# MyrtleSoftware/myrtlespeech

Measured on AMD Instinct MI355X. Metric: audio-sec/s (RTF), DS2 5xBiLSTM-1024 encoder forward + CTC greedy, 80-feature 10 s clips @ batch 32/GPU, higher is better.
Workload: dtype f16x3 (f32 split in fp16 hi+lo, 3 fp16 MFMA passes, f32 acc: LSTM, projections, conv1/2, FC1; FC2/CTC/decode f32)

## Files before the change

### include/ms_hotpath.h

```cpp
#ifndef MS_HOTPATH_H
#define MS_HOTPATH_H

#include <stddef.h>
#include <stdint.h>

#ifdef __cplusplus
extern "C" {
#endif

#define MS_ABI_VERSION 4

enum {
  MS_OK = 0,
  MS_ERR_INVALID = 1,
  MS_ERR_HIP = 2,
  MS_ERR_WORKSPACE = 3,
  MS_ERR_TIMEOUT = 4,
  MS_ERR_UNSUPPORTED = 5
};

enum { MS_CELL_LSTM = 0, MS_CELL_GRU = 1, MS_CELL_RNN_TANH = 2, MS_CELL_HARD_LSTM = 3 };

enum { MS_ACT_NONE = 0, MS_ACT_CLAMP = 1  };

int ms_abi_version(void);
const char* ms_last_error(void);


int ms_mask_time_(float* x, const int32_t* lens, int N, int inner, int T, void* stream);

size_t ms_maskconv_packed_bytes(int Cout, int Cin_g, int KF, int KT, int groups);

int ms_maskconv_pack(const float* w, void* packed, int Cout, int Cin_g, int KF, int KT, int groups, void* stream);

int ms_maskconv_forward(const float* x, const int32_t* lens, const void* packed_w, const float* bias, float* y,
                        int N, int Cin, int Fin, int Tin, int Cout, int Fout, int Tout, int KF, int KT, int SF,
                        int ST, int DF, int DT, int pad_f_l, int pad_t_l, int groups, int act, float act_lo,
                        float act_hi, void* stream);

size_t ms_maskconv_cl_packed_bytes(int Cout, int Cin, int KF, int KT);
int ms_maskconv_cl_pack(const float* w, void* packed, int Cout, int Cin, int KF, int KT, void* stream);
size_t ms_maskconv_cl_workspace_bytes(int N, int Cin, int Fin, int Tin);
int ms_maskconv_cl_forward(const float* x, const int32_t* lens, const void* packed_w, const float* bias, float* y,
                           int N, int Cin, int Fin, int Tin, int Cout, int Fout, int Tout, int KF, int KT, int SF,
                           int ST, int DF, int DT, int pad_f_l, int pad_t_l, int act, float act_lo, float act_hi,
                           void* workspace, size_t workspace_bytes, void* stream);

size_t ms_maskconv_fwin_packed_bytes(int Cout, int KF, int KT);
int ms_maskconv_fwin_pack(const float* w, void* packed, int Cout, int KF, int KT, void* stream);
size_t ms_maskconv_fwin_workspace_bytes(int N, int Tin, int KF, int SF, int Fout);
int ms_maskconv_fwin_forward(const float* x, const int32_t* lens, const void* packed_w, const float* bias, float* y, int N,
                             int Fin, int Tin, int Cout, int Fout, int Tout, int KF, int KT, int SF, int ST, int DT,
                             int pad_f_l, int pad_t_l, int act, float act_lo, float act_hi, void* workspace,
                             size_t workspace_bytes, void* stream);

size_t ms_maskconv1d_gemm_packed_bytes(int Cout, int Cin, int KT);
int ms_maskconv1d_gemm_pack(const float* w, void* packed, int Cout, int Cin, int KT, void* stream);
size_t ms_maskconv1d_gemm_workspace_bytes(int N, int Cin, int Tout, int Cout, int KT);
int ms_maskconv1d_gemm_forward(const float* x, const int32_t* lens, const void* packed, const float* bias, float* y, int N,
                               int Cin, int Tin, int Cout, int Tout, int KT, int ST, int DT, int pad_l, int act,
                               float act_lo, float act_hi, void* workspace, size_t workspace_bytes, void* stream);

int ms_nct_to_tnc(const float* x, float* y, int N, int CF, int T, void* stream);

int ms_clamp(const float* x, float* y, size_t n, float lo, float hi, void* stream);


int ms_linear_forward(const float* x, const float* w, const float* bias, float* y, int M, int K, int N, int act,
                      float act_lo, float act_hi, void* stream);

#define MS_LINEAR_FEW_ROWS 1
size_t ms_linear_splitk_workspace_bytes(int M, int K, int N, int flags);
int ms_linear_splitk_forward(const float* x, const float* w, const float* bias, float* y, int M, int K, int N, int act,
                             float act_lo, float act_hi, int flags, void* workspace, size_t workspace_bytes, void* stream);

size_t ms_linear_split_workspace_bytes(int M, int K, int N);
int ms_linear_split_forward(const float* x, const float* w, const float* bias, float* y, int M, int K, int N, int act,
                            float act_lo, float act_hi, void* workspace, size_t workspace_bytes, void* stream);

size_t ms_linear_split_packed_bytes(int K, int N);
int ms_linear_split_pack(const float* w, void* packed, int K, int N, void* stream);
int ms_linear_split_forward_packed(const float* x, const void* packed_w, const float* bias, float* y, int M, int K, int N, int act,
                                   float act_lo, float act_hi, void* workspace, size_t workspace_bytes, void* stream);


int ms_lookahead_forward(const float* x, const float* w, float* y, int N, int F, int T, int ctx, long xs_n,
                         long xs_f, long xs_t, long ys_n, long ys_f, long ys_t, int act, float act_lo,
                         float act_hi, void* stream);

int ms_lookahead_window_forward(const float* x, const float* w, float* y, int N, int F, int T_in, int T_out, int ctx,
                                long xs_n, long xs_f, long xs_t, long ys_n, long ys_f, long ys_t, int act, float act_lo,
                                float act_hi, void* stream);


int ms_rnn_padded_hidden(int cell, int H, int ndir);
size_t ms_rnn_packed_bytes(int cell, int In, int H, int ndir);
int ms_rnn_pack(int cell, int In, int H, int ndir, const float* const* w_ih_host, const float* const* w_hh_host,
                const float* const* b_ih_host, const float* const* b_hh_host, void* packed, void* stream);

size_t ms_rnn_workspace_bytes(int cell, int T, int N, int In, int H, int ndir);

int ms_rnn_layer_forward(int cell, const void* packed, const float* x, const int32_t* lens, int max_len,
                         const float* h0, const float* c0, float* out, float* hn, float* cn, int T, int N, int In,
                         int H, int ndir, void* workspace, size_t workspace_bytes, void* stream);

enum { MS_RNN_X_PLANES_IN_WS = 1, MS_RNN_OUT_PLANES_TO_WS = 2, MS_RNN_PACKED_ROWS = 4, MS_RNN_HX_PREINIT = 4096,
       MS_RNN_RECURRENCE_ONLY = 8192, MS_RNN_TIMING_SKIP_PROJECTION = 8192 ,
       MS_RNN_PROJECTION_ONLY = 16384 };
int ms_rnn_layer_chains_planes(int cell, int H, int ndir);
int ms_rnn_hx_preinit(int cell, int T, int N, int In, int H, int ndir, int max_len, int nregions, void* workspace,
                      size_t workspace_bytes, void* stream);
int ms_rnn_layer_packs_rows(int cell, int T, int N, int In, int H, int ndir);
int ms_rnn_layer_forward_ex(int cell, const void* packed, const float* x, const int32_t* lens, int max_len,
                            const float* h0, const float* c0, float* out, float* hn, float* cn, int T, int N, int In,
                            int H, int ndir, int flags, void* workspace, size_t workspace_bytes, void* stream);

int ms_rnn_layer_is_wide(int cell, int H, int ndir, int N);
int ms_rnn_stack_overlap_ok(int cell, int T, int N, int In, int H, int ndir, int nl);
int ms_rnn_stack_forward(int cell, const void* const* packed_host, const float* x, const int32_t* lens, int max_len,
                         const float* h0, const float* c0, float* out, float* hn, float* cn, int T, int N, int In, int H, int ndir,
                         int nl, int segments, void* workspace, size_t workspace_bytes, void* stream);

int ms_rnn_status(const void* workspace, void* stream);

size_t ms_rnn_debug_offset(int cell, int T, int N, int In, int H, int ndir);

int ms_gemm_set_variant(int variant);

enum {
  MS_PROF_PROJECTION = 0, MS_PROF_RECURRENCE = 1, MS_PROF_GEMM_K_LARGE = 2, MS_PROF_GEMM_K_SMALL = 3, MS_PROF_CONV = 4,
  MS_PROF_LAYOUT = 5, MS_PROF_LINEAR = 6, MS_PROF_GREEDY = 7, MS_PROF_OTHER = 8
};
#define MS_PROF_KINDS 9
int ms_prof_enable(int on);
int ms_prof_read(float* out_ms_host, int* out_n_host);

int ms_clock_probe(unsigned long long* out_dev, int samples, int spacing_us, void* stream);
// ... 105 lines not shown
```

### myrtlespeech_amd/_lib.py

```python
import ctypes
import os
import re
from ctypes import POINTER, c_char_p, c_double, c_float, c_int, c_int32, c_long, c_size_t, c_void_p

import torch

_HERE = os.path.dirname(os.path.abspath(__file__))
LIB_PATH = os.environ.get("MS_HOTPATH_LIB") or os.path.join(_HERE, "libms_hotpath.so")
HEADER_PATH = os.path.join(os.path.dirname(_HERE), "include", "ms_hotpath.h")

MS_OK = 0
ABI_VERSION = 4
ERR_NAMES = {1: "MS_ERR_INVALID", 2: "MS_ERR_HIP", 3: "MS_ERR_WORKSPACE", 4: "MS_ERR_TIMEOUT", 5: "MS_ERR_UNSUPPORTED"}

CELL_LSTM, CELL_GRU, CELL_RNN_TANH, CELL_HARD_LSTM = 0, 1, 2, 3
ACT_NONE, ACT_CLAMP = 0, 1
LINEAR_FEW_ROWS = 1
PROF_KINDS = 9

_P = c_void_p
_PP = POINTER(c_void_p)

SIGNATURES = {
    "ms_abi_version": (c_int, []),
    "ms_last_error": (c_char_p, []),
    "ms_mask_time_": (c_int, [_P, _P, c_int, c_int, c_int, _P]),
    "ms_maskconv_packed_bytes": (c_size_t, [c_int, c_int, c_int, c_int, c_int]),
    "ms_maskconv_pack": (c_int, [_P, _P, c_int, c_int, c_int, c_int, c_int, _P]),
    "ms_maskconv_forward": (c_int, [_P, _P, _P, _P, _P] + [c_int] * 17 + [c_float, c_float, _P]),
    "ms_maskconv_cl_packed_bytes": (c_size_t, [c_int, c_int, c_int, c_int]),
    "ms_maskconv_cl_pack": (c_int, [_P, _P, c_int, c_int, c_int, c_int, _P]),
    "ms_maskconv_cl_workspace_bytes": (c_size_t, [c_int, c_int, c_int, c_int]),
    "ms_maskconv_cl_forward": (c_int, [_P, _P, _P, _P, _P] + [c_int] * 16 + [c_float, c_float, _P, c_size_t, _P]),
    "ms_maskconv_fwin_packed_bytes": (c_size_t, [c_int, c_int, c_int]),
    "ms_maskconv_fwin_pack": (c_int, [_P, _P, c_int, c_int, c_int, _P]),
    "ms_maskconv_fwin_workspace_bytes": (c_size_t, [c_int, c_int, c_int, c_int, c_int]),
    "ms_maskconv_fwin_forward": (c_int, [_P, _P, _P, _P, _P] + [c_int] * 14 + [c_float, c_float, _P, c_size_t, _P]),
    "ms_maskconv1d_gemm_packed_bytes": (c_size_t, [c_int, c_int, c_int]),
    "ms_maskconv1d_gemm_pack": (c_int, [_P, _P, c_int, c_int, c_int, _P]),
    "ms_maskconv1d_gemm_workspace_bytes": (c_size_t, [c_int] * 5),
    "ms_maskconv1d_gemm_forward": (c_int, [_P, _P, _P, _P, _P] + [c_int] * 10 + [c_float, c_float, _P, c_size_t, _P]),
    "ms_nct_to_tnc": (c_int, [_P, _P, c_int, c_int, c_int, _P]),
    "ms_clamp": (c_int, [_P, _P, c_size_t, c_float, c_float, _P]),
    "ms_linear_forward": (c_int, [_P, _P, _P, _P, c_int, c_int, c_int, c_int, c_float, c_float, _P]),
    "ms_linear_splitk_workspace_bytes": (c_size_t, [c_int, c_int, c_int, c_int]),
    "ms_linear_splitk_forward": (c_int, [_P, _P, _P, _P, c_int, c_int, c_int, c_int, c_float, c_float, c_int, _P, c_size_t, _P]),
    "ms_linear_split_workspace_bytes": (c_size_t, [c_int, c_int, c_int]),
    "ms_linear_split_forward": (c_int, [_P, _P, _P, _P, c_int, c_int, c_int, c_int, c_float, c_float, _P, c_size_t, _P]),
    "ms_linear_split_packed_bytes": (c_size_t, [c_int, c_int]),
    "ms_linear_split_pack": (c_int, [_P, _P, c_int, c_int, _P]),
    "ms_linear_split_forward_packed": (c_int, [_P, _P, _P, _P, c_int, c_int, c_int, c_int, c_float, c_float, _P, c_size_t, _P]),
    "ms_lookahead_forward": (c_int, [_P, _P, _P, c_int, c_int, c_int, c_int] + [c_long] * 6 + [c_int, c_float, c_float, _P]),
    "ms_lookahead_window_forward": (c_int, [_P, _P, _P, c_int, c_int, c_int, c_int, c_int] + [c_long] * 6 + [c_int, c_float, c_float, _P]),
    "ms_rnn_packed_bytes": (c_size_t, [c_int, c_int, c_int, c_int]),
    "ms_ctc_status": (c_int, [_P, _P]),
    "ms_rnn_padded_hidden": (c_int, [c_int, c_int, c_int]),
    "ms_rnn_hx_preinit": (c_int, [c_int] * 8 + [_P, c_size_t, _P]),
    "ms_rnn_pack": (c_int, [c_int, c_int, c_int, c_int, _PP, _PP, _PP, _PP, _P, _P]),
    "ms_rnn_workspace_bytes": (c_size_t, [c_int] * 6),
    "ms_rnn_layer_forward": (c_int, [c_int, _P, _P, _P, c_int, _P, _P, _P, _P, _P] + [c_int] * 5 + [_P, c_size_t, _P]),
    "ms_rnn_layer_forward_ex": (c_int, [c_int, _P, _P, _P, c_int, _P, _P, _P, _P, _P] + [c_int] * 6 + [_P, c_size_t, _P]),
    "ms_rnn_layer_chains_planes": (c_int, [c_int, c_int, c_int]),
    "ms_rnn_layer_is_wide": (c_int, [c_int] * 4),
    "ms_rnn_stack_overlap_ok": (c_int, [c_int] * 7),
    "ms_rnn_stack_forward": (c_int, [c_int, _P, _P, _P, c_int, _P, _P, _P, _P, _P] + [c_int] * 7 + [_P, c_size_t, _P]),
    "ms_rnn_status": (c_int, [_P, _P]),
    "ms_rnn_debug_offset": (c_size_t, [c_int] * 6),
    "ms_rnn_layer_packs_rows": (c_int, [c_int] * 6),
    "ms_gemm_set_variant": (c_int, [c_int]),
    "ms_prof_enable": (c_int, [c_int]),
    "ms_prof_read": (c_int, [POINTER(c_float), POINTER(c_int)]),
    "ms_clock_probe": (c_int, [_P, c_int, c_int, _P]),
    "ms_barrier_chain_probe": (c_int, [_P, c_int, c_int, _P]),
    "ms_ctc_loss_workspace_bytes": (c_size_t, [c_int] * 4),
    "ms_ctc_loss_forward": (c_int, [_P] * 7 + [c_int] * 7 + [_P, c_size_t, _P]),
    "ms_log_softmax_axis": (c_int, [_P, _P, c_int, c_int, c_int, _P]),
    "ms_log_softmax_axis_backward": (c_int, [_P, _P, _P, c_int, c_int, c_int, _P]),
    "ms_ctc_loss_backward_workspace_bytes": (c_size_t, [c_int] * 4),
    "ms_ctc_loss_backward": (c_int, [_P] * 7 + [c_int] * 6 + [_P, c_size_t, _P]),
    "ms_ctc_greedy_decode": (c_int, [_P, _P, _P, _P, c_int, c_int, c_int, c_int, _P]),
    "ms_ctc_greedy_stream_state_bytes": (c_size_t, [c_int]),
    "ms_ctc_greedy_stream_begin": (c_int, [_P, c_int, _P]),
    "ms_ctc_greedy_stream_step": (c_int, [_P, c_int, c_int, c_int, c_int, _P, _P, _P, _P, c_int, _P, _P, c_int, _P]),
    "ms_embedding_forward": (c_int, [_P, _P, _P, c_int, c_int, c_int, _P]),
    "ms_rnnt_joint_forward": (c_int, [_P, _P, _P, _P, _P, _P, c_int, c_int, c_int, _P]),
    "ms_rnnt_topk": (c_int, [_P, _P, _P, c_int, c_int, c_int, _P]),
    "ms_ctc_beam_workspace_bytes": (c_size_t, [c_int] * 4),
    "ms_ctc_beam_decode": (c_int, [_P, _P, _P, _P, c_int, c_int, c_int, c_int, c_int, c_float, c_int, _P, c_int, c_int,
                                   _P, c_int, _P, _P, _P, _P, c_size_t, _P]),
    "ms_ctc_beam_decode_rows": (c_int, [_P, _P, _P, _P, c_int, c_int, c_int, c_int, c_int, c_float, c_int, _P, c_int, c_int,
                                        c_int, c_int, _P, c_int, _P, _P, _P, _P, c_size_t, _P]),
    "ms_ngram_lm_table_check": (c_int, [_P, c_size_t]),
    "ms_ngram_lm_score": (c_int, [_P, _P, c_size_t, _P, _P, _P, c_int, c_int, c_int, _P]),
    "ms_ctc_beam_lm_workspace_bytes": (c_size_t, [c_int] * 5),
    "ms_ctc_beam_decode_lm": (c_int, [_P, _P, _P, _P, c_int, c_int, c_int, c_int, c_int, c_float, c_int, _P, c_int, c_int,
                                      c_int, c_int, _P, _P, c_size_t, c_int, _P, _P, _P, _P, c_size_t, _P]),
    "ms_rnnt_decode_workspace_bytes": (c_size_t, [c_int] * 10),
    "ms_rnnt_decode": (c_int, [_P, _P, _P, _PP, _PP, _PP, _PP, _P, _P, _P, _P, _P, _P] + [c_int] * 10 + [_P, c_size_t, _P]),
    "ms_mfcc_workspace_bytes": (c_size_t, [c_int] * 5),
    "ms_mfcc_forward": (c_int, [_P] * 7 + [c_int] * 7 + [c_float, _P, c_size_t, _P]),
    "ms_mfcc_legacy_forward": (c_int, [_P] * 7 + [c_int] * 8 + [c_double, _P]),
    "ms_standardize_workspace_bytes": (c_size_t, [c_int]),
    "ms_standardize_forward": (c_int, [_P, _P, _P, c_int, c_int, c_int, _P, c_size_t, _P]),
    "ms_context_frames_forward": (c_int, [_P, _P, _P, c_int, c_int, c_int, c_int, _P]),
    "ms_spec_augment_": (c_int, [_P, _P, _P] + [c_int] * 6 + [_P]),
}

_lib = None


def header_symbols():
    with open(HEADER_PATH) as f:
        text = re.sub(r"/\*.*?\*/", "", f.read(), flags=re.S)
    return sorted(set(re.findall(r"\b(ms_[a-z0-9_]+)\s*\(", text)))


# ... 194 lines not shown
```

### myrtlespeech_amd/csrc/conv_cl.hip

```cpp
#include <algorithm>
#include <type_traits>

#include "common.h"

namespace {

typedef unsigned u32x4 __attribute__((ext_vector_type(4)));
typedef unsigned u32x2 __attribute__((ext_vector_type(2)));
typedef __bf16 bf16x8 __attribute__((ext_vector_type(8)));
typedef _Float16 f16x8 __attribute__((ext_vector_type(8)));

constexpr int CL_F = 2;

struct ClP {
  int N, Cin, Fin, Tin, Cout, Fout, Tout, KF, KT, SF, ST, DF, DT, pad_f, pad_t;
  int KG;
  int PW;
  int co_tiles;
  int act;
  float lo, hi;
  int FP;
};

__device__ __forceinline__ unsigned bf16b(float x) { return (unsigned)__builtin_bit_cast(unsigned short, (__bf16)x); }
// ... 71 lines not shown
      const bool frow = (fo0 + f) < p.Fout && (WIN || (fin >= 0 && fin < p.Fin));
      const size_t rbase = ((size_t)n * p.Fin + (frow && !WIN ? fin : 0)) * p.Tin;
      for (int i = tid; i < ngran; i += 256) {
        const int q = i / p.KG, kg = i - q * p.KG;
        const int tin = tin0 + q;
        u32x4 vh = {0u, 0u, 0u, 0u}, vl = {0u, 0u, 0u, 0u};
        if (frow && tin >= 0 && tin < len) {
          if (WIN) {
            const int boff = (int)((((size_t)n * p.Tin + tin) * p.FP + (size_t)(fo0 + f) * p.SF + kg * 8) * 2);
            vh = __builtin_amdgcn_raw_buffer_load_b128(xh_rsrc, boff, 0, 0);
            if (!F16) vl = __builtin_amdgcn_raw_buffer_load_b128(xl_rsrc, boff, 0, 0);
          } else {
            const size_t off = (rbase + tin) * p.Cin + kg * 8;
            vh = *reinterpret_cast<const u32x4*>(xh + off);
            if (!F16) vl = *reinterpret_cast<const u32x4*>(xl + off);
          }
        }
        *reinterpret_cast<u32x4*>(Ph + f * row_bytes + (kg * p.PW + q) * 16) = vh;
        if (!F16) *reinterpret_cast<u32x4*>(Pl + f * row_bytes + (kg * p.PW + q) * 16) = vl;
      }
    }
    const int taps_per_stage = (p.KT + 1) / 2;
    for (int kt0 = 0; kt0 < p.KT; kt0 += taps_per_stage) {
      const int ntap = min(taps_per_stage, p.KT - kt0);
      if (kt0 > 0) __syncthreads();
      {
        const int ng = ntap * p.KG * 32;
        for (int i = tid; i < ng; i += 256) {
          const int co = i & 31, rest = i >> 5;
          const size_t src = ((((size_t)kf * p.KT + kt0) * p.KG + rest) * cout_pad + tile * 32 + co) * 8;
          *reinterpret_cast<u32x4*>(Wh + i * 16) = *reinterpret_cast<const u32x4*>(wp + src);
          if (!F16) *reinterpret_cast<u32x4*>(Wl + i * 16) = *reinterpret_cast<const u32x4*>(wp + wplane + src);
        }
      }
      __syncthreads();
      for (int ktl = 0; ktl < ntap; ++ktl) {
        const int tq = (wt * 32 + l31) * p.ST + (kt0 + ktl) * p.DT;
        for (int s = 0; s < p.KG / 2; ++s) {
          const int kg = 2 * s + half;
          const int woff = ((ktl * p.KG + kg) * 32 + l31) * 16;
          const u32x4 ah = *reinterpret_cast<const u32x4*>(Wh + woff);
          u32x4 al = ah;
          if (!F16) al = *reinterpret_cast<const u32x4*>(Wl + woff);
#pragma unroll
          for (int f = 0; f < CL_F; ++f) {
            const int poff = (wf * CL_F + f) * row_bytes + (kg * p.PW + tq) * 16;
            const u32x4 bh = *reinterpret_cast<const u32x4*>(Ph + poff);
            if (F16) {
              acc[f] = __builtin_amdgcn_mfma_f32_32x32x16_f16(__builtin_bit_cast(f16x8, ah), __builtin_bit_cast(f16x8, bh), acc[f], 0, 0, 0);
            } else {
              const u32x4 bl = *reinterpret_cast<const u32x4*>(Pl + poff);
              acc[f] = ms::mfma_32x32x16<HM>(ah, bh, acc[f]);
              acc[f] = ms::mfma_32x32x16<HM>(al, bh, acc[f]);
              acc[f] = ms::mfma_32x32x16<HM>(ah, bl, acc[f]);
            }
          }
        }
      }
    }
    __syncthreads();
  }

  const int t = t0 + wt * 32 + l31;
  const float winv = scale_word[1];
  if (t < p.Tout) {
#pragma unroll
    for (int f = 0; f < CL_F; ++f) {
      const int fo = fo0 + wf * CL_F + f;
      if (fo >= p.Fout) continue;
#pragma unroll
      for (int r = 0; r < 16; ++r) {
        const int co = tile * 32 + ms::mfma32_row(r, lane);
        if (co < p.Cout) {
          float v = acc[f][r] * winv + (bias ? bias[co] : 0.f);
          if (p.act == MS_ACT_CLAMP) v = fminf(fmaxf(v, p.lo), p.hi);
          y[(((size_t)n * p.Cout + co) * p.Fout + fo) * p.Tout + t] = v;
        }
      }
    }
  }
}


constexpr int SH_RB = 12;
constexpr int SH_KT = 11;

template <int P>
__global__ __launch_bounds__(256, 1) void maskconv_cl_short_kernel(const unsigned short* __restrict__ xh,
                                                                   const unsigned short* __restrict__ xl,
                                                                   const int32_t* __restrict__ lens,
                                                                   const unsigned short* __restrict__ wp,
                                                                   const float* __restrict__ bias, float* __restrict__ y, ClP p,
                                                                   int RB, int RIN, const float* __restrict__ scale_word) {
  constexpr bool F16 = ms::prec_one_plane(P), HM = P == ms::PREC_F16X3;
  const float winv = scale_word[1];
  extern __shared__ __attribute__((aligned(16))) char lds[];
  const int tid = threadIdx.x, lane = tid & 63, wave = __builtin_amdgcn_readfirstlane(tid >> 6);
  const int c16 = lane & 15, q = lane >> 4;
  const int fo0 = blockIdx.x * RB, cb = blockIdx.y, n = blockIdx.z;
  const int PW = p.PW;
  const int row_bytes = PW * 64;
  char* Ph = lds;
  char* Pl = lds + (size_t)RIN * row_bytes;
  const int len = lens ? min(lens[n], p.Tin) : p.Tin;
  const int fin_lo = fo0 * p.SF - p.pad_f;

  for (int i = tid; i < RIN * PW * 4; i += 256) {
    const int kg = i & 3, rq = i >> 2;
    const int r = rq / PW, fq = rq - r * PW;
    const int fin = fin_lo + r, tin = fq - p.pad_t;
    u32x4 vh = {0u, 0u, 0u, 0u}, vl = {0u, 0u, 0u, 0u};
    if (fin >= 0 && fin < p.Fin && tin >= 0 && tin < len) {
      const size_t off = (((size_t)n * p.Fin + fin) * p.Tin + tin) * 32 + kg * 8;
      vh = *reinterpret_cast<const u32x4*>(xh + off);
      if (!F16) vl = *reinterpret_cast<const u32x4*>(xl + off);
    }
    *reinterpret_cast<u32x4*>(Ph + r * row_bytes + fq * 64 + kg * 16) = vh;
    if (!F16) *reinterpret_cast<u32x4*>(Pl + r * row_bytes + fq * 64 + kg * 16) = vl;
  }
  __syncthreads();

  ms::f32x4 acc[SH_RB];
#pragma unroll
  for (int i = 0; i < SH_RB; ++i) acc[i] = ms::f32x4{0.f, 0.f, 0.f, 0.f};
  const int cout_pad = p.co_tiles * 32;
  const size_t wplane = (size_t)p.KF * p.KT * 4 * cout_pad * 8;
  const unsigned short* wa = wp + (size_t)q * cout_pad * 8 + (cb * 16 + c16) * 8;
  const size_t tap_stride = (size_t)4 * cout_pad * 8;
  u32x4 fh[2][SH_KT], fl[2][SH_KT];
  auto load_row = [&](auto set, int kf) {
#pragma unroll
    for (int kt = 0; kt < SH_KT; ++kt)
      if (kt < p.KT) {
        const unsigned short* src = wa + (size_t)(kf * p.KT + kt) * tap_stride;
        fh[set][kt] = *reinterpret_cast<const u32x4*>(src);
        if (!F16) fl[set][kt] = *reinterpret_cast<const u32x4*>(src + wplane);
      }
  };
  auto compute_row = [&](auto set, int kf) {
#pragma unroll
    for (int i = 0; i < SH_RB; ++i) {
      const int fo = fo0 + i;
      const int fin = fo * p.SF - p.pad_f + kf * p.DF;
      if (i < RB && fo < p.Fout && fin >= 0 && fin < p.Fin) {
        const int rbase = (fin - fin_lo) * row_bytes + c16 * 64 + q * 16;
#pragma unroll
        for (int kt = 0; kt < SH_KT; ++kt)
          if (kt < p.KT) {
            const u32x4 bh = *reinterpret_cast<const u32x4*>(Ph + rbase + kt * 64);
            if (F16) {
              acc[i] = __builtin_amdgcn_mfma_f32_16x16x32_f16(__builtin_bit_cast(f16x8, fh[set][kt]), __builtin_bit_cast(f16x8, bh), acc[i], 0, 0, 0);
            } else {
              const u32x4 bl = *reinterpret_cast<const u32x4*>(Pl + rbase + kt * 64);
              acc[i] = ms::mfma_16x16x32<HM>(fh[set][kt], bh, acc[i]);
              acc[i] = ms::mfma_16x16x32<HM>(fl[set][kt], bh, acc[i]);
              acc[i] = ms::mfma_16x16x32<HM>(fh[set][kt], bl, acc[i]);
            }
          }
      }
    }
  };
  constexpr std::integral_constant<int, 0> S0{};
  constexpr std::integral_constant<int, 1> S1{};
  if (wave < p.KF) load_row(S0, wave);
  for (int kf = wave; kf < p.KF; kf += 8) {
    if (kf + 4 < p.KF) load_row(S1, kf + 4);
// ... 102 lines not shown
    const int kg = (i / ((size_t)8 * cout_pad)) % KG;
    const int kt = i / ((size_t)8 * cout_pad * KG);
    const int kf = kg * 8 + e;
    float x = 0.f;
    if (co < Cout && kf < KF) x = w[((size_t)co * KF + kf) * KT + kt] * wscale;
    unsigned h, l;
    split_by_prec(x, prec, h, l);
    packed[i] = (unsigned short)h;
    packed[plane + i] = (unsigned short)l;
  }
}

int conv_cl_plan(ClP& p, size_t* lds) {
  const size_t wbytes = (size_t)2 * ((p.KT + 1) / 2) * p.KG * 32 * 16;
  if ((long)p.N * p.co_tiles > 65535) return 0;
  for (int wf : {p.Tout <= 48 ? 4 : 1, 1}) {
    const int tt = 128 / wf, rf = CL_F * wf;
    p.PW = (tt - 1) * p.ST + (p.KT - 1) * p.DT + 1;
    *lds = (size_t)2 * rf * p.KG * p.PW * 16 + wbytes;
    if (*lds <= 160 * 1024 && ms::cdiv(p.Fout, rf) <= 65535) return wf;
  }
  return 0;
}

template <bool WIN>
int conv_cl_launch(const ClP& p, int wf, size_t lds, const unsigned short* xh, const unsigned short* xl, const int32_t* lens,
                   const void* packed_w, const float* bias, float* y, hipStream_t stream, const float* scale_word) {
  static ms::DeviceOnce attr_once;
  if (attr_once.need()) {
#define MS_CL_ATTR(PP)                                                                                                                     \
    MS_HIP(hipFuncSetAttribute((const void*)maskconv_cl_kernel<PP, WIN, 1>, hipFuncAttributeMaxDynamicSharedMemorySize, 160 * 1024));   \
    MS_HIP(hipFuncSetAttribute((const void*)maskconv_cl_kernel<PP, WIN, 4>, hipFuncAttributeMaxDynamicSharedMemorySize, 160 * 1024));
    MS_CL_ATTR(ms::PREC_BF16X3) MS_CL_ATTR(ms::PREC_F16) MS_CL_ATTR(ms::PREC_F16X3)
#undef MS_CL_ATTR
    attr_once.done();
  }
  const int prec = ms::split_mode();
  const int tt = 128 / wf, rf = CL_F * wf;
  dim3 grid(ms::cdiv(p.Tout, tt), ms::cdiv(p.Fout, rf), p.N * p.co_tiles);
  const unsigned short* wq = (const unsigned short*)packed_w;
#define MS_CL_LAUNCH(WF_)                                                                                                             \
  if (prec == ms::PREC_F16) hipLaunchKernelGGL((maskconv_cl_kernel<ms::PREC_F16, WIN, WF_>), grid, dim3(256), lds, stream, xh, xl, lens, wq, bias, y, p, scale_word); \
  else if (prec == ms::PREC_F16X3) hipLaunchKernelGGL((maskconv_cl_kernel<ms::PREC_F16X3, WIN, WF_>), grid, dim3(256), lds, stream, xh, xl, lens, wq, bias, y, p, scale_word); \
  else hipLaunchKernelGGL((maskconv_cl_kernel<ms::PREC_BF16X3, WIN, WF_>), grid, dim3(256), lds, stream, xh, xl, lens, wq, bias, y, p, scale_word);
  if (wf == 4) { MS_CL_LAUNCH(4) } else { MS_CL_LAUNCH(1) }
#undef MS_CL_LAUNCH
  MS_LAUNCH_CHECK();
  return MS_OK;
}

inline int fwin_kfp(int KF) { return ms::cdiv(KF, 16) * 16; }
inline int fwin_fp(int KF, int SF, int Fout) { return ms::cdiv((Fout - 1) * SF + fwin_kfp(KF), 32) * 32; }

}

static size_t fwin_plane_bytes(int Cout, int KF, int KT) {
  return ms::align_up((size_t)2 * KT * (fwin_kfp(KF) / 8) * (ms::cdiv(Cout, 32) * 32) * 8 * sizeof(unsigned short), 256);
}
extern "C" size_t ms_maskconv_fwin_packed_bytes(int Cout, int KF, int KT) {
  if (Cout <= 0 || KF <= 0 || KT <= 0) return 0;
  return fwin_plane_bytes(Cout, KF, KT) + 256;
}

extern "C" int ms_maskconv_fwin_pack(const float* w, void* packed, int Cout, int KF, int KT, void* stream) {
  MS_REQUIRE(w && packed, "null pointer");
  MS_REQUIRE(Cout > 0 && KF > 0 && KT > 0, "bad shape");
  const int cout_pad = ms::cdiv(Cout, 32) * 32, KG = fwin_kfp(KF) / 8;
  const size_t plane = (size_t)KT * KG * cout_pad * 8;
  const int blocks = (int)std::min<size_t>((plane + 255) / 256, 2048);
  float* scale_word = (float*)((char*)packed + fwin_plane_bytes(Cout, KF, KT));
  const int rc = ms::weight_scale_launch(w, (size_t)Cout * KF * KT, scale_word, ms::split_mode(), (hipStream_t)stream);
  if (rc != MS_OK) return rc;
  hipLaunchKernelGGL(conv_fwin_pack_kernel, dim3(blocks), dim3(256), 0, (hipStream_t)stream, w, (unsigned short*)packed, Cout,
                     KF, KT, KG, cout_pad, ms::split_mode(), scale_word);
  MS_LAUNCH_CHECK();
  return MS_OK;
}

extern "C" size_t ms_maskconv_fwin_workspace_bytes(int N, int Tin, int KF, int SF, int Fout) {
  if (N <= 0 || Tin <= 0 || KF <= 0 || SF <= 0 || Fout <= 0) return 0;
  return ms::align_up((size_t)N * Tin * fwin_fp(KF, SF, Fout) * 4, 256);
}

extern "C" int ms_maskconv_fwin_forward(const float* x, const int32_t* lens, const void* packed_w, const float* bias, float* y,
                                        int N, int Fin, int Tin, int Cout, int Fout, int Tout, int KF, int KT, int SF, int ST,
                                        int DT, int pad_f_l, int pad_t_l, int act, float act_lo, float act_hi, void* workspace,
                                        size_t workspace_bytes, void* stream_) {
  ms::ProfScope prof_span(MS_PROF_CONV, (hipStream_t)stream_);
  MS_REQUIRE(x && packed_w && y && workspace, "null pointer");
  MS_REQUIRE(N > 0 && Fin > 0 && Tin > 0 && Cout > 0 && Fout > 0 && Tout > 0, "bad shape");
  MS_REQUIRE(KF > 0 && KT > 0 && SF > 0 && ST > 0 && DT > 0 && pad_f_l >= 0 && pad_t_l >= 0, "bad kernel");
  MS_REQUIRE(SF % 2 == 0, "feature stride must be even (4-byte aligned window loads)");
  MS_REQUIRE(act == MS_ACT_NONE || act == MS_ACT_CLAMP, "bad act");
  if (workspace_bytes < ms_maskconv_fwin_workspace_bytes(N, Tin, KF, SF, Fout)) {
    ms::set_error("ms_maskconv_fwin_forward: workspace too small");
    return MS_ERR_WORKSPACE;
  }
  hipStream_t stream = (hipStream_t)stream_;
  ClP p;
  p.N = N; p.Cin = fwin_kfp(KF); p.Fin = 1; p.Tin = Tin; p.Cout = Cout; p.Fout = Fout; p.Tout = Tout; p.KF = 1; p.KT = KT;
  p.SF = SF; p.ST = ST; p.DF = 1; p.DT = DT; p.pad_f = 0; p.pad_t = pad_t_l; p.KG = p.Cin / 8;
  p.co_tiles = ms::cdiv(Cout, 32);
  p.act = act; p.lo = act_lo; p.hi = act_hi;
  p.FP = fwin_fp(KF, SF, Fout);
  size_t lds = 0;
  const int wf = conv_cl_plan(p, &lds);
  if (wf == 0 || (size_t)N * Tin * p.FP * 2 >= ((size_t)1 << 31)) {
    ms::set_error("ms_maskconv_fwin_forward: shape outside the LDS / grid budget");
    return MS_ERR_UNSUPPORTED;
  }
  unsigned short* xh = (unsigned short*)workspace;
  unsigned short* xl = xh + (size_t)N * Tin * p.FP;
  const int prec = ms::split_mode();
  const bool f16 = prec == ms::PREC_F16;
  hipLaunchKernelGGL(ft_to_tf_split_kernel, dim3(ms::cdiv(Tin, 32), ms::cdiv(p.FP, 32), N), dim3(32, 8), 0, stream, x, xh, xl,
                     Fin, Tin, p.FP, pad_f_l, prec);
  MS_LAUNCH_CHECK();
  return conv_cl_launch<true>(p, wf, lds, xh, xl, lens, packed_w, bias, y, stream,
                              (const float*)((const char*)packed_w + fwin_plane_bytes(Cout, KF, KT)));
}

static size_t cl_plane_bytes(int Cout, int Cin, int KF, int KT) {
  return ms::align_up((size_t)2 * KF * KT * (Cin / 8) * (ms::cdiv(Cout, 32) * 32) * 8 * sizeof(unsigned short), 256);
}
extern "C" size_t ms_maskconv_cl_packed_bytes(int Cout, int Cin, int KF, int KT) {
  if (Cout <= 0 || Cin <= 0 || Cin % 16 || KF <= 0 || KT <= 0) return 0;
  return cl_plane_bytes(Cout, Cin, KF, KT) + 256;
}

extern "C" int ms_maskconv_cl_pack(const float* w, void* packed, int Cout, int Cin, int KF, int KT, void* stream) {
  MS_REQUIRE(w && packed, "null pointer");
  MS_REQUIRE(Cout > 0 && Cin > 0 && Cin % 16 == 0 && KF > 0 && KT > 0, "bad shape (Cin must be a multiple of 16)");
  const int cout_pad = ms::cdiv(Cout, 32) * 32;
  const size_t plane = (size_t)KF * KT * (Cin / 8) * cout_pad * 8;
  const int blocks = (int)std::min<size_t>((plane + 255) / 256, 2048);
  float* scale_word = (float*)((char*)packed + cl_plane_bytes(Cout, Cin, KF, KT));
  const int rc = ms::weight_scale_launch(w, (size_t)Cout * Cin * KF * KT, scale_word, ms::split_mode(), (hipStream_t)stream);
  if (rc != MS_OK) return rc;
  hipLaunchKernelGGL(conv_cl_pack_kernel, dim3(blocks), dim3(256), 0, (hipStream_t)stream, w, (unsigned short*)packed, Cout,
                     Cin, KF, KT, cout_pad, ms::split_mode(), scale_word);
  MS_LAUNCH_CHECK();
  return MS_OK;
}

extern "C" size_t ms_maskconv_cl_workspace_bytes(int N, int Cin, int Fin, int Tin) {
  if (N <= 0 || Cin <= 0 || Fin <= 0 || Tin <= 0) return 0;
  return ms::align_up((size_t)N * Cin * Fin * Tin * 4, 256);
}

extern "C" int ms_maskconv_cl_forward(const float* x, const int32_t* lens, const void* packed_w, const float* bias, float* y,
                                      int N, int Cin, int Fin, int Tin, int Cout, int Fout, int Tout, int KF, int KT,
                                      int SF, int ST, int DF, int DT, int pad_f_l, int pad_t_l, int act, float act_lo,
                                      float act_hi, void* workspace, size_t workspace_bytes, void* stream_) {
  ms::ProfScope prof_span(MS_PROF_CONV, (hipStream_t)stream_);
  MS_REQUIRE(x && packed_w && y && workspace, "null pointer");
  MS_REQUIRE(N > 0 && Cin > 0 && Cin % 16 == 0 && Fin > 0 && Tin > 0 && Cout > 0 && Fout > 0 && Tout > 0, "bad shape");
  MS_REQUIRE(KF > 0 && KT > 0 && SF > 0 && ST > 0 && DF > 0 && DT > 0 && pad_f_l >= 0 && pad_t_l >= 0, "bad kernel");
  MS_REQUIRE(act == MS_ACT_NONE || act == MS_ACT_CLAMP, "bad act");
  if (workspace_bytes < ms_maskconv_cl_workspace_bytes(N, Cin, Fin, Tin)) {
    ms::set_error("ms_maskconv_cl_forward: workspace too small");
    return MS_ERR_WORKSPACE;
  }
  hipStream_t stream = (hipStream_t)stream_;
  ClP p;
  p.N = N; p.Cin = Cin; p.Fin = Fin; p.Tin = Tin; p.Cout = Cout; p.Fout = Fout; p.Tout = Tout; p.KF = KF; p.KT = KT;
  p.SF = SF; p.ST = ST; p.DF = DF; p.DT = DT; p.pad_f = pad_f_l; p.pad_t = pad_t_l; p.KG = Cin / 8;
  p.co_tiles = ms::cdiv(Cout, 32);
  p.act = act; p.lo = act_lo; p.hi = act_hi;
  p.FP = 0;
  size_t lds = 0;
  const int wf = conv_cl_plan(p, &lds);
  if (wf == 0) {
    ms::set_error("ms_maskconv_cl_forward: shape outside the LDS / grid budget");
    return MS_ERR_UNSUPPORTED;
  }
  const float* scale_word = (const float*)((const char*)packed_w + cl_plane_bytes(Cout, Cin, KF, KT));
  unsigned short* xh = (unsigned short*)workspace;
  unsigned short* xl = xh + (size_t)N * Cin * Fin * Tin;
  MS_REQUIRE(N * Fin <= 65535, "N*Fin exceeds grid limits");
  const int prec = ms::split_mode();
  const bool f16 = prec == ms::PREC_F16;
  hipLaunchKernelGGL(nchw_to_cl_split_kernel, dim3(ms::cdiv(Tin, 32), ms::cdiv(Cin, 32), N * Fin), dim3(32, 8), 0, stream, x,
                     xh, xl, Cin, Fin, Tin, prec);
  MS_LAUNCH_CHECK();
  {
    int RB = 0, RIN = 0;
    size_t slds = 0;
    if (conv_cl_short_plan(p, f16, &RB, &RIN, &slds)) {
      static ms::DeviceOnce attr_once;
      if (attr_once.need()) {
        MS_HIP(hipFuncSetAttribute((const void*)maskconv_cl_short_kernel<ms::PREC_BF16X3>, hipFuncAttributeMaxDynamicSharedMemorySize, 160 * 1024));
        MS_HIP(hipFuncSetAttribute((const void*)maskconv_cl_short_kernel<ms::PREC_F16>, hipFuncAttributeMaxDynamicSharedMemorySize, 160 * 1024));
        MS_HIP(hipFuncSetAttribute((const void*)maskconv_cl_short_kernel<ms::PREC_F16X3>, hipFuncAttributeMaxDynamicSharedMemorySize, 160 * 1024));
        attr_once.done();
      }
      ClP ps = p;
      ps.PW = Tout + KT - 1;
      const dim3 grid(ms::cdiv(Fout, RB), ms::cdiv(Cout, 16), N);
      const unsigned short* wq = (const unsigned short*)packed_w;
      auto kern = prec == ms::PREC_F16 ? maskconv_cl_short_kernel<ms::PREC_F16>
                  : prec == ms::PREC_F16X3 ? maskconv_cl_short_kernel<ms::PREC_F16X3> : maskconv_cl_short_kernel<ms::PREC_BF16X3>;
      hipLaunchKernelGGL(kern, grid, dim3(256), slds, stream, xh, xl, lens, wq, bias, y, ps, RB, RIN, scale_word);
      MS_LAUNCH_CHECK();
      return MS_OK;
    }
  }
  return conv_cl_launch<false>(p, wf, lds, xh, xl, lens, packed_w, bias, y, stream, scale_word);
}
```

Before: 27000.

## Add register-prefetch pipelined conv kernels for channels-last and freq-window convs

Adds two new MFMA conv kernels. The first stages each kf slice of input and weights through registers, so the global loads for slice kf+1 are issued while slice kf is computed from LDS. The second stages the whole freq-window tile at once using buffer loads and a stride-deinterleaved LDS layout, loading weights in two halves to fit the LDS budget. The aim is to hide global-load latency and cut per-tap barrier stalls in conv1/conv2, at the cost of higher register and LDS pressure (one block per CU for the fwin kernel) plus new eligibility plans and env switches.

```diff
diff --git a/include/ms_hotpath.h b/include/ms_hotpath.h
--- a/include/ms_hotpath.h
+++ b/include/ms_hotpath.h
@@ -45,6 +45,8 @@
                            int N, int Cin, int Fin, int Tin, int Cout, int Fout, int Tout, int KF, int KT, int SF,
                            int ST, int DF, int DT, int pad_f_l, int pad_t_l, int act, float act_lo, float act_hi,
                            void* workspace, size_t workspace_bytes, void* stream);
+int ms_maskconv_cl_pipelined(int N, int Cin, int Fin, int Tin, int Cout, int Fout, int Tout, int KF, int KT, int SF, int ST,
+                             int DF, int DT);
 
 size_t ms_maskconv_fwin_packed_bytes(int Cout, int KF, int KT);
 int ms_maskconv_fwin_pack(const float* w, void* packed, int Cout, int KF, int KT, void* stream);
@@ -53,6 +55,7 @@
                              int Fin, int Tin, int Cout, int Fout, int Tout, int KF, int KT, int SF, int ST, int DT,
                              int pad_f_l, int pad_t_l, int act, float act_lo, float act_hi, void* workspace,
                              size_t workspace_bytes, void* stream);
+int ms_maskconv_fwin_batched(int N, int Tin, int Cout, int Fout, int Tout, int KF, int KT, int SF, int ST, int DT);
 
 size_t ms_maskconv1d_gemm_packed_bytes(int Cout, int Cin, int KT);
 int ms_maskconv1d_gemm_pack(const float* w, void* packed, int Cout, int Cin, int KT, void* stream);
diff --git a/myrtlespeech_amd/_lib.py b/myrtlespeech_amd/_lib.py
--- a/myrtlespeech_amd/_lib.py
+++ b/myrtlespeech_amd/_lib.py
@@ -32,6 +32,8 @@
     "ms_maskconv_cl_pack": (c_int, [_P, _P, c_int, c_int, c_int, c_int, _P]),
     "ms_maskconv_cl_workspace_bytes": (c_size_t, [c_int, c_int, c_int, c_int]),
     "ms_maskconv_cl_forward": (c_int, [_P, _P, _P, _P, _P] + [c_int] * 16 + [c_float, c_float, _P, c_size_t, _P]),
+    "ms_maskconv_cl_pipelined": (c_int, [c_int] * 13),
+    "ms_maskconv_fwin_batched": (c_int, [c_int] * 10),
     "ms_maskconv_fwin_packed_bytes": (c_size_t, [c_int, c_int, c_int]),
     "ms_maskconv_fwin_pack": (c_int, [_P, _P, c_int, c_int, c_int, _P]),
     "ms_maskconv_fwin_workspace_bytes": (c_size_t, [c_int, c_int, c_int, c_int, c_int]),
diff --git a/myrtlespeech_amd/csrc/conv_cl.hip b/myrtlespeech_amd/csrc/conv_cl.hip
--- a/myrtlespeech_amd/csrc/conv_cl.hip
+++ b/myrtlespeech_amd/csrc/conv_cl.hip
@@ -177,6 +177,373 @@
 }
 
 
+constexpr int PL_XS = 5;
+constexpr int PL_WS = 6;
+
+template <int P>
+__global__ __launch_bounds__(256, 2) void maskconv_cl_pipe_kernel(const unsigned short* __restrict__ xh,
+                                                                  const unsigned short* __restrict__ xl,
+                                                                  const int32_t* __restrict__ lens,
+                                                                  const unsigned short* __restrict__ wp,
+                                                                  const float* __restrict__ bias, float* __restrict__ y, ClP p,
+                                                                  const float* __restrict__ scale_word) {
+  constexpr bool F16 = ms::prec_one_plane(P), HM = P == ms::PREC_F16X3;
+  constexpr int TT = 128, RF = CL_F;
+  extern __shared__ __attribute__((aligned(16))) char lds[];
+  const int row_bytes = p.KG * p.PW * 16;
+  char* Ph = lds;
+  char* Pl = lds + RF * row_bytes;
+  char* Wh = lds + 2 * RF * row_bytes;
+  const int wrow = p.KT * p.KG * 32;
+  char* Wl = Wh + wrow * 16;
+
+  const int tid = threadIdx.x, lane = tid & 63, wave = tid >> 6;
+  const int l31 = lane & 31, half = lane >> 5;
+  const int t0 = blockIdx.x * TT;
+  const int fo0 = blockIdx.y * RF;
+  const int n = blockIdx.z / p.co_tiles, tile = blockIdx.z % p.co_tiles;
+  const int len = lens ? min(lens[n], p.Tin) : p.Tin;
+  const int cout_pad = p.co_tiles * 32;
+  const size_t wplane = (size_t)p.KF * p.KT * p.KG * cout_pad * 8;
+
+  ms::f32x16 acc[CL_F];
+#pragma unroll
+  for (int f = 0; f < CL_F; ++f)
+#pragma unroll
+    for (int r = 0; r < 16; ++r) acc[f][r] = 0.f;
+
+  const int tin0 = t0 * p.ST - p.pad_t;
+  const int ngran = p.KG * p.PW;
+  int x_lds[PL_XS];
+  int x_src[PL_XS];
+  int x_row[PL_XS];
+#pragma unroll
+  for (int sl = 0; sl < PL_XS; ++sl) {
+    const int j = sl * 256 + tid;
+    const int f = j / ngran, i = j - f * ngran;
+    const int q = i / p.KG, kg = i - q * p.KG;
+    const int tin = tin0 + q;
+    x_row[sl] = f;
+    x_lds[sl] = j < RF * ngran ? f * row_bytes + (kg * p.PW + q) * 16 : -1;
+    x_src[sl] = (j < RF * ngran && tin >= 0 && tin < len) ? tin * p.Cin + kg * 8 : -1;
+  }
+  const size_t row_elems = (size_t)p.Tin * p.Cin;
+  const size_t wkf = (size_t)wrow / 32 * cout_pad * 8;
+
+  u32x4 rxh[PL_XS], rxl[PL_XS], rwh[PL_WS], rwl[PL_WS];
+  auto request = [&](int kf) {
+#pragma unroll
+    for (int sl = 0; sl < PL_XS; ++sl) {
+      const int f = x_row[sl];
+      const int fin = (fo0 + f) * p.SF - p.pad_f + kf * p.DF;
+      rxh[sl] = u32x4{0u, 0u, 0u, 0u};
+      rxl[sl] = u32x4{0u, 0u, 0u, 0u};
+      if (x_src[sl] >= 0 && (fo0 + f) < p.Fout && fin >= 0 && fin < p.Fin) {
+        const size_t off = ((size_t)n * p.Fin + fin) * row_elems + x_src[sl];
+        rxh[sl] = *reinterpret_cast<const u32x4*>(xh + off);
+        if (!F16) rxl[sl] = *reinterpret_cast<const u32x4*>(xl + off);
+      }
+    }
+#pragma unroll
+    for (int sl = 0; sl < PL_WS; ++sl) {
+      const int i = sl * 256 + tid;
+      if (i < wrow) {
+        const int co = i & 31, rest = i >> 5;
+        const size_t src = kf * wkf + ((size_t)rest * cout_pad + tile * 32 + co) * 8;
+        rwh[sl] = *reinterpret_cast<const u32x4*>(wp + src);
+        if (!F16) rwl[sl] = *reinterpret_cast<const u32x4*>(wp + wplane + src);
+      }
+    }
+  };
+  auto publish = [&]() {
+#pragma unroll
+    for (int sl = 0; sl < PL_XS; ++sl)
+      if (x_lds[sl] >= 0) {
+        *reinterpret_cast<u32x4*>(Ph + x_lds[sl]) = rxh[sl];
+        if (!F16) *reinterpret_cast<u32x4*>(Pl + x_lds[sl]) = rxl[sl];
+      }
+#pragma unroll
+    for (int sl = 0; sl < PL_WS; ++sl) {
+      const int i = sl * 256 + tid;
+      if (i < wrow) {
+        *reinterpret_cast<u32x4*>(Wh + i * 16) = rwh[sl];
+        if (!F16) *reinterpret_cast<u32x4*>(Wl + i * 16) = rwl[sl];
+      }
+    }
+  };
+
+  struct Ops { u32x4 ah, al, bh[CL_F], bl[CL_F]; };
+  const int S = p.KG / 2;
+  const int nstep = p.KT * S;
+  const int a_lane = (half * 32 + l31) * 16;
+  const int b_lane = (half * p.PW + (wave * 32 + l31) * p.ST) * 16;
+  auto fetch = [&](Ops& o, int i, int kt, int s) {
+    const int woff = i * 1024 + a_lane;
+    o.ah = *reinterpret_cast<const u32x4*>(Wh + woff);
+    o.al = o.ah;
+    if (!F16) o.al = *reinterpret_cast<const u32x4*>(Wl + woff);
+    const int poff = b_lane + (2 * s * p.PW + kt * p.DT) * 16;
+#pragma unroll
+    for (int f = 0; f < CL_F; ++f) {
+      o.bh[f] = *reinterpret_cast<const u32x4*>(Ph + f * row_bytes + poff);
+      if (!F16) o.bl[f] = *reinterpret_cast<const u32x4*>(Pl + f * row_bytes + poff);
+    }
+  };
+  auto mfmas = [&](const Ops& o) {
+#pragma unroll
+    for (int f = 0; f < CL_F; ++f) {
+      if (F16) {
+        acc[f] = __builtin_amdgcn_mfma_f32_32x32x16_f16(__builtin_bit_cast(f16x8, o.ah), __builtin_bit_cast(f16x8, o.bh[f]), acc[f], 0, 0, 0);
+      } else {
+        acc[f] = ms::mfma_32x32x16<HM>(o.ah, o.bh[f], acc[f]);
+        acc[f] = ms::mfma_32x32x16<HM>(o.al, o.bh[f], acc[f]);
+        acc[f] = ms::mfma_32x32x16<HM>(o.ah, o.bl[f], acc[f]);
+      }
+    }
+  };
+
+  request(0);
+  for (int kf = 0; kf < p.KF; ++kf) {
+    publish();
+    __syncthreads();
+    if (kf + 1 < p.KF) request(kf + 1);
+    Ops o0, o1;
+    int kt = 0, s = 0;
+    auto advance = [&](int i) {
+      if (i < nstep) { const bool wrap = s + 1 == S; s = wrap ? 0 : s + 1; kt += wrap; }
+      return min(i, nstep - 1);
+    };
+    fetch(o0, 0, kt, s);
+    for (int i = 0; i + 2 <= nstep; i += 2) {
+      const int i1 = advance(i + 1);
+      fetch(o1, i1, kt, s);
+      mfmas(o0);
+      const int i2 = advance(i + 2);
+      fetch(o0, i2, kt, s);
+      mfmas(o1);
+    }
+    if (nstep & 1) mfmas(o0);
+    __syncthreads();
+  }
+
+  const int t = t0 + wave * 32 + l31;
+  const float winv = scale_word[1];
+  if (t < p.Tout) {
+#pragma unroll
+    for (int f = 0; f < CL_F; ++f) {
+      const int fo = fo0 + f;
+      if (fo >= p.Fout) continue;
+#pragma unroll
+      for (int r = 0; r < 16; ++r) {
+        const int co = tile * 32 + ms::mfma32_row(r, lane);
+        if (co < p.Cout) {
+          float v = acc[f][r] * winv + (bias ? bias[co] : 0.f);
+          if (p.act == MS_ACT_CLAMP) v = fminf(fmaxf(v, p.lo), p.hi);
+          y[(((size_t)n * p.Cout + co) * p.Fout + fo) * p.Tout + t] = v;
+        }
+      }
+    }
+  }
+}
+
+int conv_cl_pipe_plan(const ClP& p, bool f16, size_t* lds) {
+  const char* sw = getenv("MS_CONV_PIPE");
+  if (sw && sw[0] == '0') return 0;
+  if (p.FP != 0 || p.KG % 2 || p.Tout <= 48) return 0;
+  const size_t xgran = (size_t)CL_F * p.KG * p.PW, wgran = (size_t)p.KT * p.KG * 32;
+  if (xgran > (size_t)256 * PL_XS || wgran > (size_t)256 * PL_WS) return 0;
+  if ((size_t)p.Tin * p.Cin >= ((size_t)1 << 31)) return 0;
+  (void)f16;
+  *lds = 2 * (xgran + wgran) * 16;
+  return *lds <= 80 * 1024;
+}
+
+constexpr int FW_XS = 25;
+constexpr int FW_WS = 9;
+static_assert(CL_F == 2, "maskconv_fwin_batch_kernel tells its two staged rows apart with one comparison");
+
+template <int P>
+__global__ __launch_bounds__(256, 1) void maskconv_fwin_batch_kernel(const unsigned short* __restrict__ xh,
+                                                                     const unsigned short* __restrict__ xl,
+                                                                     const int32_t* __restrict__ lens,
+                                                                     const unsigned short* __restrict__ wp,
+                                                                     const float* __restrict__ bias, float* __restrict__ y,
+                                                                     ClP p, const float* __restrict__ scale_word) {
+  constexpr bool F16 = ms::prec_one_plane(P), HM = P == ms::PREC_F16X3;
+  constexpr int TT = 128, RF = CL_F;
+  extern __shared__ __attribute__((aligned(16))) char lds[];
+  const int PWS = (p.PW + p.ST - 1) / p.ST;
+  const int PWL = PWS * p.ST;
+  const int row_bytes = p.KG * PWL * 16;
+  char* Ph = lds;
+  char* Pl = lds + RF * row_bytes;
+  char* Wh = lds + 2 * RF * row_bytes;
+  const int taps_per_stage = (p.KT + 1) / 2;
+  const int whalf = taps_per_stage * p.KG * 32;
+  const int wall = p.KT * p.KG * 32;
+  char* Wl = Wh + whalf * 16;
+
+  const int tid = threadIdx.x, lane = tid & 63, wave = tid >> 6;
+  const int l31 = lane & 31, half = lane >> 5;
+  const int t0 = blockIdx.x * TT;
+  const int fo0 = blockIdx.y * RF;
+  const int n = blockIdx.z / p.co_tiles, tile = blockIdx.z % p.co_tiles;
+  const int len = lens ? min(lens[n], p.Tin) : p.Tin;
+  const int cout_pad = p.co_tiles * 32;
+  const size_t wplane = (size_t)wall / 32 * cout_pad * 8;
+
+  ms::f32x16 acc[CL_F];
+#pragma unroll
+  for (int f = 0; f < CL_F; ++f)
+#pragma unroll
+    for (int r = 0; r < 16; ++r) acc[f][r] = 0.f;
+
+  const int tin0 = t0 * p.ST - p.pad_t;
+  const int ngran = p.KG * p.PW;
+  const unsigned plane_bytes = (unsigned)((size_t)p.N * p.Tin * p.FP * 2);
+  const __amdgpu_buffer_rsrc_t xh_rsrc = __builtin_amdgcn_make_buffer_rsrc(const_cast<unsigned short*>(xh), 0, plane_bytes, 0x00020000);
+  const __amdgpu_buffer_rsrc_t xl_rsrc = __builtin_amdgcn_make_buffer_rsrc(const_cast<unsigned short*>(xl), 0, plane_bytes, 0x00020000);
+
+  u32x4 rxh[FW_XS], rxl[FW_XS], rwh[FW_WS], rwl[FW_WS];
+  int x_lds[FW_XS];
+  const float rkg = 1.f / (float)p.KG, rst = 1.f / (float)p.ST;
+#pragma unroll
+  for (int sl = 0; sl < FW_XS; ++sl) {
+    const int j = sl * 256 + tid;
+    const int f = j >= ngran ? 1 : 0, i = j - f * ngran;
+    const int q = (int)(((float)i + 0.5f) * rkg), kg = i - q * p.KG;
+    const int qd = (int)(((float)q + 0.5f) * rst), qm = q - qd * p.ST;
+    const int tin = tin0 + q;
+    const bool have = j < RF * ngran;
+    x_lds[sl] = have ? f * row_bytes + (kg * PWL + qm * PWS + qd) * 16 : -1;
+    rxh[sl] = u32x4{0u, 0u, 0u, 0u};
+    rxl[sl] = u32x4{0u, 0u, 0u, 0u};
+    if (have && (fo0 + f) < p.Fout && tin >= 0 && tin < len) {
+      const int boff = (int)((((size_t)n * p.Tin + tin) * p.FP + (size_t)(fo0 + f) * p.SF + kg * 8) * 2);
+      rxh[sl] = __builtin_amdgcn_raw_buffer_load_b128(xh_rsrc, boff, 0, 0);
+      if (!F16) rxl[sl] = __builtin_amdgcn_raw_buffer_load_b128(xl_rsrc, boff, 0, 0);
+    }
+  }
+#pragma unroll
+  for (int sl = 0; sl < FW_WS; ++sl) {
+    const int i = sl * 256 + tid;
+    if (i < wall) {
+      const int co = i & 31, rest = i >> 5;
+      const size_t src = ((size_t)rest * cout_pad + tile * 32 + co) * 8;
+      rwh[sl] = *reinterpret_cast<const u32x4*>(wp + src);
+      if (!F16) rwl[sl] = *reinterpret_cast<const u32x4*>(wp + wplane + src);
+    }
+  }
+  auto publish_w = [&](int second) {
+#pragma unroll
+    for (int sl = 0; sl < FW_WS; ++sl) {
+      const int i = sl * 256 + tid;
+      if (i < wall && (i >= whalf) == (second != 0)) {
+        const int il = i - (second ? whalf : 0);
+        *reinterpret_cast<u32x4*>(Wh + il * 16) = rwh[sl];
+        if (!F16) *reinterpret_cast<u32x4*>(Wl + il * 16) = rwl[sl];
+      }
+    }
+  };
+#pragma unroll
+  for (int sl = 0; sl < FW_XS; ++sl)
+    if (x_lds[sl] >= 0) {
+      *reinterpret_cast<u32x4*>(Ph + x_lds[sl]) = rxh[sl];
+      if (!F16) *reinterpret_cast<u32x4*>(Pl + x_lds[sl]) = rxl[sl];
+    }
+  publish_w(0);
+  __syncthreads();
+
+  struct Ops { u32x4 ah, al, bh[CL_F], bl[CL_F]; };
+  const int S = p.KG / 2;
+  const int dq = p.DT / p.ST, dm = p.DT - dq * p.ST;
+  const int a_lane = (half * 32 + l31) * 16;
+  const int b_lane = (half * PWL + wave * 32 + l31) * 16;
+  int s = 0, km = 0, kq = 0;
+  auto advance = [&]() {
+    if (++s == S) {
+      s = 0; km += dm; kq += dq;
+      if (km >= p.ST) { km -= p.ST; ++kq; }
+    }
+  };
+  auto fetch = [&](Ops& o, int i) {
+    const int woff = i * 1024 + a_lane;
+    o.ah = *reinterpret_cast<const u32x4*>(Wh + woff);
+    o.al = o.ah;
+    if (!F16) o.al = *reinterpret_cast<const u32x4*>(Wl + woff);
+    const int poff = b_lane + (2 * s * PWL + km * PWS + kq) * 16;
+#pragma unroll
+    for (int f = 0; f < CL_F; ++f) {
+      o.bh[f] = *reinterpret_cast<const u32x4*>(Ph + f * row_bytes + poff);
+      if (!F16) o.bl[f] = *reinterpret_cast<const u32x4*>(Pl + f * row_bytes + poff);
+    }
+  };
+  auto mfmas = [&](const Ops& o) {
+#pragma unroll
+    for (int f = 0; f < CL_F; ++f) {
+      if (F16) {
+        acc[f] = __builtin_amdgcn_mfma_f32_32x32x16_f16(__builtin_bit_cast(f16x8, o.ah), __builtin_bit_cast(f16x8, o.bh[f]), acc[f], 0, 0, 0);
+      } else {
+        acc[f] = ms::mfma_32x32x16<HM>(o.ah, o.bh[f], acc[f]);
+        acc[f] = ms::mfma_32x32x16<HM>(o.al, o.bh[f], acc[f]);
+        acc[f] = ms::mfma_32x32x16<HM>(o.ah, o.bl[f], acc[f]);
+      }
+    }
+  };
+  auto run_taps = [&](int ntap) {
+    const int nstep = ntap * S;
+    Ops o0, o1;
+    fetch(o0, 0);
+    for (int i = 0; i + 2 <= nstep; i += 2) {
+      advance();
+      fetch(o1, i + 1);
+      mfmas(o0);
+      if (i + 2 < nstep) advance();
+      fetch(o0, min(i + 2, nstep - 1));
+      mfmas(o1);
+    }
+    if (nstep & 1) mfmas(o0);
+    advance();
+  };
+  run_taps(taps_per_stage);
+  if (p.KT > taps_per_stage) {
+    __syncthreads();
+    publish_w(1);
+    __syncthreads();
+    run_taps(p.KT - taps_per_stage);
+  }
+
+  const int t = t0 + wave * 32 + l31;
+  const float winv = scale_word[1];
+  if (t < p.Tout) {
+#pragma unroll
+    for (int f = 0; f < CL_F; ++f) {
+      const int fo = fo0 + f;
+      if (fo >= p.Fout) continue;
+#pragma unroll
+      for (int r = 0; r < 16; ++r) {
+        const int co = tile * 32 + ms::mfma32_row(r, lane);
+        if (co < p.Cout) {
+          float v = acc[f][r] * winv + (bias ? bias[co] : 0.f);
+          if (p.act == MS_ACT_CLAMP) v = fminf(fmaxf(v, p.lo), p.hi);
+          y[(((size_t)n * p.Cout + co) * p.Fout + fo) * p.Tout + t] = v;
+        }
+      }
+    }
+  }
+}
+
+int conv_fwin_batch_plan(const ClP& p, size_t* lds) {
+  const char* sw = getenv("MS_CONV_FWIN_BATCH");
+  if (sw && sw[0] == '0') return 0;
+  if (p.FP == 0 || p.KG % 2 || p.Tout <= 48 || p.KF != 1) return 0;
+  const size_t xgran = (size_t)CL_F * p.KG * p.PW, wgran = (size_t)p.KT * p.KG * 32;
+  if (xgran > (size_t)256 * FW_XS || wgran > (size_t)256 * FW_WS || p.KG > 64 || p.ST > 64) return 0;
+  const size_t pwl = (size_t)ms::cdiv(p.PW, p.ST) * p.ST;
+  *lds = 2 * ((size_t)CL_F * p.KG * pwl + (size_t)((p.KT + 1) / 2) * p.KG * 32) * 16;
+  return *lds <= 160 * 1024;
+}
+
 constexpr int SH_RB = 12;
 constexpr int SH_KT = 11;
 
@@ -445,6 +812,20 @@
   return ms::align_up((size_t)N * Tin * fwin_fp(KF, SF, Fout) * 4, 256);
 }
 
+extern "C" int ms_maskconv_fwin_batched(int N, int Tin, int Cout, int Fout, int Tout, int KF, int KT, int SF, int ST, int DT) {
+  if (N <= 0 || Tin <= 0 || Cout <= 0 || Fout <= 0 || Tout <= 0 || KF <= 0 || KT <= 0 || SF <= 0 || SF % 2 || ST <= 0 || DT <= 0)
+    return 0;
+  ClP p;
+  p.N = N; p.Cin = fwin_kfp(KF); p.Fin = 1; p.Tin = Tin; p.Cout = Cout; p.Fout = Fout; p.Tout = Tout; p.KF = 1; p.KT = KT;
+  p.SF = SF; p.ST = ST; p.DF = 1; p.DT = DT; p.pad_f = 0; p.pad_t = 0; p.KG = p.Cin / 8;
+  p.co_tiles = ms::cdiv(Cout, 32);
+  p.act = MS_ACT_NONE; p.lo = p.hi = 0.f;
+  p.FP = fwin_fp(KF, SF, Fout);
+  size_t lds = 0;
+  if ((size_t)N * Tin * p.FP * 2 >= ((size_t)1 << 31)) return 0;
+  return conv_cl_plan(p, &lds) == 1 && conv_fwin_batch_plan(p, &lds);
+}
+
 extern "C" int ms_maskconv_fwin_forward(const float* x, const int32_t* lens, const void* packed_w, const float* bias, float* y,
                                         int N, int Fin, int Tin, int Cout, int Fout, int Tout, int KF, int KT, int SF, int ST,
                                         int DT, int pad_f_l, int pad_t_l, int act, float act_lo, float act_hi, void* workspace,
@@ -475,12 +856,28 @@
   unsigned short* xh = (unsigned short*)workspace;
   unsigned short* xl = xh + (size_t)N * Tin * p.FP;
   const int prec = ms::split_mode();
-  const bool f16 = prec == ms::PREC_F16;
   hipLaunchKernelGGL(ft_to_tf_split_kernel, dim3(ms::cdiv(Tin, 32), ms::cdiv(p.FP, 32), N), dim3(32, 8), 0, stream, x, xh, xl,
                      Fin, Tin, p.FP, pad_f_l, prec);
   MS_LAUNCH_CHECK();
-  return conv_cl_launch<true>(p, wf, lds, xh, xl, lens, packed_w, bias, y, stream,
-                              (const float*)((const char*)packed_w + fwin_plane_bytes(Cout, KF, KT)));
+  const float* scale_word = (const float*)((const char*)packed_w + fwin_plane_bytes(Cout, KF, KT));
+  size_t blds = 0;
+  if (wf == 1 && conv_fwin_batch_plan(p, &blds)) {
+    static ms::DeviceOnce attr_once;
+    if (attr_once.need()) {
+      MS_HIP(hipFuncSetAttribute((const void*)maskconv_fwin_batch_kernel<ms::PREC_BF16X3>, hipFuncAttributeMaxDynamicSharedMemorySize, 160 * 1024));
+      MS_HIP(hipFuncSetAttribute((const void*)maskconv_fwin_batch_kernel<ms::PREC_F16>, hipFuncAttributeMaxDynamicSharedMemorySize, 160 * 1024));
+      MS_HIP(hipFuncSetAttribute((const void*)maskconv_fwin_batch_kernel<ms::PREC_F16X3>, hipFuncAttributeMaxDynamicSharedMemorySize, 160 * 1024));
+      attr_once.done();
+    }
+    const dim3 grid(ms::cdiv(Tout, 128), ms::cdiv(Fout, CL_F), N * p.co_tiles);
+    const unsigned short* wq = (const unsigned short*)packed_w;
+    auto kern = prec == ms::PREC_F16 ? maskconv_fwin_batch_kernel<ms::PREC_F16>
+                : prec == ms::PREC_F16X3 ? maskconv_fwin_batch_kernel<ms::PREC_F16X3> : maskconv_fwin_batch_kernel<ms::PREC_BF16X3>;
+    hipLaunchKernelGGL(kern, grid, dim3(256), blds, stream, xh, xl, lens, wq, bias, y, p, scale_word);
+    MS_LAUNCH_CHECK();
+    return MS_OK;
+  }
+  return conv_cl_launch<true>(p, wf, lds, xh, xl, lens, packed_w, bias, y, stream, scale_word);
 }
 
 static size_t cl_plane_bytes(int Cout, int Cin, int KF, int KT) {
@@ -509,6 +906,21 @@
 extern "C" size_t ms_maskconv_cl_workspace_bytes(int N, int Cin, int Fin, int Tin) {
   if (N <= 0 || Cin <= 0 || Fin <= 0 || Tin <= 0) return 0;
   return ms::align_up((size_t)N * Cin * Fin * Tin * 4, 256);
+}
+
+extern "C" int ms_maskconv_cl_pipelined(int N, int Cin, int Fin, int Tin, int Cout, int Fout, int Tout, int KF, int KT, int SF,
+                                        int ST, int DF, int DT) {
+  if (N <= 0 || Cin <= 0 || Cin % 16 || Fin <= 0 || Tin <= 0 || Cout <= 0 || Fout <= 0 || Tout <= 0 || KF <= 0 || KT <= 0 ||
+      SF <= 0 || ST <= 0 || DF <= 0 || DT <= 0)
+    return 0;
+  ClP p;
+  p.N = N; p.Cin = Cin; p.Fin = Fin; p.Tin = Tin; p.Cout = Cout; p.Fout = Fout; p.Tout = Tout; p.KF = KF; p.KT = KT;
+  p.SF = SF; p.ST = ST; p.DF = DF; p.DT = DT; p.pad_f = 0; p.pad_t = 0; p.KG = Cin / 8;
+  p.co_tiles = ms::cdiv(Cout, 32);
+  p.act = MS_ACT_NONE; p.lo = p.hi = 0.f;
+  p.FP = 0;
+  size_t lds = 0;
+  return conv_cl_plan(p, &lds) == 1 && conv_cl_pipe_plan(p, ms::split_mode() == ms::PREC_F16, &lds);
 }
 
 extern "C" int ms_maskconv_cl_forward(const float* x, const int32_t* lens, const void* packed_w, const float* bias, float* y,
@@ -568,5 +980,22 @@
       return MS_OK;
     }
   }
+  size_t plds = 0;
+  if (wf == 1 && conv_cl_pipe_plan(p, f16, &plds)) {
+    static ms::DeviceOnce attr_once;
+    if (attr_once.need()) {
+      MS_HIP(hipFuncSetAttribute((const void*)maskconv_cl_pipe_kernel<ms::PREC_BF16X3>, hipFuncAttributeMaxDynamicSharedMemorySize, 80 * 1024));
+      MS_HIP(hipFuncSetAttribute((const void*)maskconv_cl_pipe_kernel<ms::PREC_F16>, hipFuncAttributeMaxDynamicSharedMemorySize, 80 * 1024));
+      MS_HIP(hipFuncSetAttribute((const void*)maskconv_cl_pipe_kernel<ms::PREC_F16X3>, hipFuncAttributeMaxDynamicSharedMemorySize, 80 * 1024));
+      attr_once.done();
+    }
+    const dim3 grid(ms::cdiv(Tout, 128), ms::cdiv(Fout, CL_F), N * p.co_tiles);
+    const unsigned short* wq = (const unsigned short*)packed_w;
+    auto kern = prec == ms::PREC_F16 ? maskconv_cl_pipe_kernel<ms::PREC_F16>
+                : prec == ms::PREC_F16X3 ? maskconv_cl_pipe_kernel<ms::PREC_F16X3> : maskconv_cl_pipe_kernel<ms::PREC_BF16X3>;
+    hipLaunchKernelGGL(kern, grid, dim3(256), plds, stream, xh, xl, lens, wq, bias, y, p, scale_word);
+    MS_LAUNCH_CHECK();
+    return MS_OK;
+  }
   return conv_cl_launch<false>(p, wf, lds, xh, xl, lens, packed_w, bias, y, stream, scale_word);
 }
```

Result: faster. 27690, median of 5 (+2.6%).
